# toposware/schnorr-sig

Measured on AMD Instinct MI355X. Metric: Schnorr verifications/sec, 2^20-sig batch, 1/2/4/8 MI355X; bit-exact vs CPU, higher is better.
Workload: dtype u64

## Files before the change

schnorr-sig_amd/csrc/fp6.hpp:

```cpp
#pragma once
#include "fp.hpp"

namespace ssa {

#if defined(__HIP_DEVICE_COMPILE__) && !defined(SSA_NO_F6_ASM)
#define SSA_F6_ASM 1
#include "fp6_asm.inc"
#endif

struct fp6 {
    u64 c[6];
};

SSA_DEV fp6 f6_zero() {
    fp6 r;
#pragma unroll
    for (int i = 0; i < 6; i++) r.c[i] = 0ull;
    return r;
}
SSA_DEV fp6 f6_one() {
    fp6 r = f6_zero();
    r.c[0] = 1ull;
    return r;
}
// ... 125 lines not shown
}

SSA_FN fp6 f6_sqr_flat(u64 a0, u64 a1, u64 a2_, u64 a3, u64 a4, u64 a5) {
    fp6 a;
    a.c[0] = a0; a.c[1] = a1; a.c[2] = a2_; a.c[3] = a3; a.c[4] = a4; a.c[5] = a5;
    u64 a2[6], a7[6], a14[6];
    f6_sqr_scale(a.c, a2, a7, a14);
#ifdef SSA_F6_ASM
    fp6 r;
    f6_sqr_core_asm(a.c, a2, a7, a14, r.c);
    return r;
#else
    fp6 r;
#pragma unroll
    for (int k = 0; k < 6; k++) {
        fp_acc s;
        bool first = true;
#pragma unroll
        for (int i = 0; i <= k / 2; i++) {
            int j = k - i;
            u64 y = (i == j) ? a.c[j] : a2[j];
            if (first) {
                acc_init(s, a.c[i], y);
                first = false;
            } else {
                acc_mac(s, a.c[i], y);
            }
        }
#pragma unroll
        for (int i = k + 1; i <= (k + 6) / 2; i++) {
            int j = k + 6 - i;
            if (j > 5) continue;
            u64 y = (i == j) ? a7[j] : a14[j];
            acc_mac(s, a.c[i], y);
        }
        r.c[k] = acc_reduce(s);
    }
    return r;
#endif
}
SSA_DEV fp6 f6_sqr(const fp6 &a) { return f6_sqr_flat(a.c[0], a.c[1], a.c[2], a.c[3], a.c[4], a.c[5]); }

SSA_DEV fp6 f6_sqr_inl(const fp6 &a) {
#ifdef SSA_F6_ASM
    u64 a2[6], a7[6], a14[6];
    f6_sqr_scale(a.c, a2, a7, a14);
    fp6 r;
    f6_sqr_core_asm(a.c, a2, a7, a14, r.c);
    return r;
#else
    return f6_sqr(a);
#endif
}

SSA_DEV void f6_sqr_prescale(const fp6 &a, u64 (&a2)[6], u64 (&a7)[6], u64 (&a14)[6]) {
    f6_sqr_scale(a.c, a2, a7, a14);
}
SSA_DEV void f6_mul_prescale(const fp6 &b, u64 (&b7)[6]) {
    b7[0] = 0ull;
#pragma unroll
    for (int j = 1; j < 6; j++) b7[j] = fp_mul_small(b.c[j], 7u);
}
SSA_DEV fp6 f6_sqr_sub2(const fp6 &a, const fp6 &x, const fp6 &y) {
#ifdef SSA_F6_ASM
    u64 a2[6], a7[6], a14[6];
    f6_sqr_prescale(a, a2, a7, a14);
    fp6 r;
    f6_sqr_sub2_core_asm(a.c, a2, a7, a14, x.c, y.c, r.c);
    return r;
#else
    return f6_sub(f6_sub(f6_sqr(a), x), y);
#endif
}
SSA_DEV fp6 f6_sqr_subx_sub2y(const fp6 &a, const fp6 &x, const fp6 &y) {
#ifdef SSA_F6_ASM
    u64 a2[6], a7[6], a14[6];
    f6_sqr_prescale(a, a2, a7, a14);
    fp6 r;
    f6_sqr_subx_sub2y_core_asm(a.c, a2, a7, a14, x.c, y.c, r.c);
    return r;
#else
    return f6_sub(f6_sub(f6_sqr(a), x), f6_dbl(y));
#endif
}
SSA_DEV fp6 f6_sqr_add3x(const fp6 &a, const fp6 &x) {
#ifdef SSA_F6_ASM
    u64 a2[6], a7[6], a14[6];
    f6_sqr_prescale(a, a2, a7, a14);
    fp6 r;
    f6_sqr_add3x_core_asm(a.c, a2, a7, a14, x.c, r.c);
    return r;
#else
    return f6_add(f6_sqr(a), f6_add(f6_dbl(x), x));
#endif
}
SSA_DEV fp6 f6_sqr_sub4x(const fp6 &a, const fp6 &x) {
#ifdef SSA_F6_ASM
    u64 a2[6], a7[6], a14[6];
    f6_sqr_prescale(a, a2, a7, a14);
    fp6 r;
    f6_sqr_sub4x_core_asm(a.c, a2, a7, a14, x.c, r.c);
    return r;
#else
    return f6_sub(f6_sqr(a), f6_dbl(f6_dbl(x)));
#endif
}
// ... 110 lines not shown
```

schnorr-sig_amd/csrc/ssa_api.hip:

```cpp
#define SSA_KERNELS_DEFINE 1
#include "ssa_ctx.hpp"
#include "ssa_keycache.hpp"
#include "ssa_keyed.hpp"

#include <sys/random.h>

#include <atomic>
#include <climits>
#include <functional>
#include <initializer_list>
#include <memory>
#include <mutex>
#include <thread>

static const unsigned char k_default_params[SSA_PARAMS_LENGTH] = {
#include "../params/params_default.inc"
};

extern "C" const char *ssa_strerror(int rc) {
    switch (rc) {
        case SSA_OK: return "ok";
        case SSA_INVALID_PUBLIC_KEY: return "The public key is not an element of the prime subgroup.";
        case SSA_INVALID_SIGNATURE: return "The signature is invalid or was incorrectly computed.";
        case SSA_MALFORMED: return "malformed input (the reference would panic)";
// ... 431 lines not shown
    if (int rc = check_msgs(mv, n)) return rc;
    if (n == 0) return 0;
    HIP_TRY(hipSetDevice(ctx->device));
    return timed_launch(ctx, "ssa_k_hash", [&] {
        hipLaunchKernelGGL(ssa_k_hash, dim3(grid_for(n, 256)), dim3(256), 0, ctx->stream, ctx->d_params,
                           d_sigs, d_pks, mv, n, (u64 *)nullptr, d_digests_out, (const u32 *)nullptr, 0u);
    });
}

extern "C" int ssa_rescue_hash_many_device(ssa_ctx *ctx, const uint64_t *d_felts, uint32_t felts_per_row,
                                           size_t n, uint64_t *d_digests_out) {
    if (!ctx || (n && (!d_digests_out || (felts_per_row && !d_felts)))) return SSA_ERR_ARG;
    if (n == 0) return 0;
    HIP_TRY(hipSetDevice(ctx->device));
    return timed_launch(ctx, "ssa_k_rescue", [&] {
        hipLaunchKernelGGL(ssa_k_rescue, dim3(grid_for(n, 256)), dim3(256), 0, ctx->stream, ctx->d_params,
                           (const u64 *)d_felts, felts_per_row, n, (u64 *)d_digests_out);
    });
}

int ssa_internal_hash_chunk(ssa_ctx *ctx, hipStream_t hs, const DevBatch &b, size_t cnt, uint64_t *d_h) {
    hipLaunchKernelGGL(ssa_k_hash, dim3(grid_for(cnt, 256)), dim3(256), 0, hs, ctx->d_params, b.sigs, b.pks, b.msgs, cnt,
                       (u64 *)d_h, (u8 *)nullptr, (const u32 *)nullptr, 0u);
    HIP_TRY(hipGetLastError());
    return 0;
}

int ssa_internal_hash_scalars(ssa_ctx *ctx, const DevBatch &b, size_t n) {
    if (ctx->ws_h.reserve(n * 4 * sizeof(u64))) return SSA_ERR_HIP;
    return timed_launch(ctx, "ssa_k_hash", [&] {
        hipLaunchKernelGGL(ssa_k_hash, dim3(grid_for(n, 256)), dim3(256), 0, ctx->stream, ctx->d_params,
                           b.sigs, b.pks, b.msgs, n, (u64 *)ctx->ws_h.p, (u8 *)nullptr, (const u32 *)nullptr, 0u);
    });
}

struct TailKnobs {
    unsigned pieces, gens, waves, block, min_main;
    bool uniform, reversed;
};
static TailPlan tail_plan_of(const TailKnobs &kn, size_t cnt, uint32_t flags) {
    const TailKnobs *ctx = &kn;
    TailPlan tp{};
    const bool torsion = (flags & SSA_FLAG_CHECK_TORSION) != 0;
    tp.whole[0] = 0u | 2u | 4u | ((u32)LADDER_STEPS_Q << 16);
    tp.whole[1] = 1u | 2u | 4u | ((u32)LADDER_STEPS << 16);
    const u32 n_groups = (u32)((cnt + 63) / 64);
    const unsigned cap = torsion ? (unsigned)VP_MAX - 1u : (unsigned)VP_MAX;
    const unsigned want = ctx->pieces < cap ? ctx->pieces : cap;
    const u32 tail0 = ctx->gens * ctx->waves;
    if (want < 2 || ctx->block != 256 || tail0 == 0 || n_groups < tail0 + ctx->min_main * ctx->waves) return tp;
    const u32 main_groups = ((n_groups - tail0) / 4u) * 4u;
    tp.main_blocks = main_groups / 4u;
    tp.tail_groups = ((n_groups - main_groups + 3u) / 4u) * 4u;
    const double DBL = 2642.0, ADD = 3738.0, TABLE = 57000.0, TAIL = 45000.0;
    struct Step { int pass, it; double cost; };
    std::vector<Step> steps;
    for (int pass = torsion ? 0 : 1; pass < 2; pass++)
        for (int it = 0; it < (pass == 0 ? LADDER_STEPS_Q : LADDER_STEPS); it++)
            steps.push_back({pass, it, (pass == 0 ? (double)QNAF_GAP[it + 1] : 5.0) * DBL + ADD});
    double total = TABLE + TAIL;
    for (const Step &st : steps) total += st.cost;
    std::vector<double> target;
    double frac = 0.0, f = 0.5;
    for (unsigned k = 0; k + 1 < want; k++) {
        frac += ctx->uniform ? 1.0 / (double)want : f;
        if (k + 2 < want) f *= 0.5;
        target.push_back(total * frac);
    }
    std::vector<std::pair<size_t, size_t>> pieces;
    size_t cur = 0, tix = 0;
    double acc = TABLE;
    for (size_t idx = 0; idx < steps.size(); idx++) {
        bool cut = false;
        if (idx > cur) {
            if (steps[idx].pass != steps[idx - 1].pass) cut = true;
            else if (tix < target.size() && acc + steps[idx].cost * 0.5 >= target[tix]) cut = true;
        }
        if (cut) {
            pieces.push_back({cur, idx});
            cur = idx;
        }
        while (tix < target.size() && acc + steps[idx].cost * 0.5 >= target[tix]) tix++;
        acc += steps[idx].cost;
    }
    pieces.push_back({cur, steps.size()});
    if (pieces.size() < 2 || pieces.size() > (size_t)VP_MAX) return tp;
    for (const auto &pc : pieces) {
        const int pass = steps[pc.first].pass, lo = steps[pc.first].it, hi = steps[pc.second - 1].it + 1;
        const int n_steps = pass == 0 ? LADDER_STEPS_Q : LADDER_STEPS;
        tp.ph[tp.n_pieces++] = (u32)pass | (lo == 0 ? 2u : 0u) | (hi == n_steps ? 4u : 0u) | ((u32)lo << 8) | ((u32)hi << 16);
    }
    tp.reversed = ctx->reversed ? 1u : 0u;
    return tp;
}
static TailPlan tail_plan(const ssa_ctx *ctx, size_t cnt, uint32_t flags) {
    return tail_plan_of({ctx->knobs.tail_pieces, ctx->knobs.tail_gens, ctx->knobs.verify_waves, ctx->knobs.verify_block, ctx->knobs.tail_min_main,
                         ctx->knobs.tail_uniform, ctx->knobs.tail_reversed}, cnt, flags);
}

extern "C" int ssa_debug_tail_plan(unsigned waves, unsigned pieces, unsigned gens, int uniform, unsigned min_main, size_t n,
                                   uint32_t flags, uint32_t out[14]) {
    if (!out) return SSA_ERR_ARG;
    const TailPlan tp = tail_plan_of({pieces, gens, waves, 256u, min_main, uniform != 0, false}, n, flags);
    out[0] = tp.n_pieces;
    out[1] = tp.tail_groups;
    out[2] = tp.main_blocks;
    out[3] = tp.n_pieces ? tail_grid_blocks(tp) : (uint32_t)((n + 255) / 256);
    for (int k = 0; k < VP_MAX; k++) out[4 + k] = tp.ph[k];
    out[12] = tp.whole[0];
    out[13] = tp.whole[1];
    return 0;
}

static int verify_slices(ssa_ctx *ctx, const DevBatch &b, const u64 *d_h, size_t n, uint32_t flags, uint8_t *d_status_out,
                         unsigned long long *d_fail) {
    return for_dev_slices(b, n, ctx->knobs.lane_slice, [&](size_t lo, size_t cnt, const DevBatch &s) {
        const TailPlan tp = tail_plan(ctx, cnt, flags);
        unsigned blocks = grid_for(cnt, ctx->knobs.verify_block);
        if (tp.n_pieces) {
            if (ctx->tail_done.reserve(2 * (size_t)tp.tail_groups * sizeof(u32)) ||
                ctx->tail_park.reserve((size_t)tp.tail_groups * PARK_WORDS * 64 * sizeof(u64)))
                return SSA_ERR_HIP;
            HIP_TRY(hipMemsetAsync(ctx->tail_done.p, 0, 2 * (size_t)tp.tail_groups * sizeof(u32), ctx->stream));
            blocks = tail_grid_blocks(tp);
        }
        return timed_launch(ctx, "ssa_k_verify", [&] {
            hipLaunchKernelGGL(ssa_k_verify, dim3(blocks), dim3(ctx->knobs.verify_block), 0,
                               ctx->stream, s.sigs, s.pks, s.pk_inf, d_h + 4 * lo, (const u64 *)ctx->d_gtab,
                               (u64 *)ctx->ws_tab.p, cnt, flags, d_status_out + lo, d_fail, tp, (u32 *)ctx->tail_done.p,
                               (u64 *)ctx->tail_park.p);
        });
    });
}

int ssa_internal_verify_hashed(ssa_ctx *ctx, const DevBatch &b, const uint64_t *d_h, size_t n, uint32_t flags,
                               uint8_t *d_status_out, unsigned long long *d_fail) {
    const size_t slice = ctx->knobs.lane_slice < n ? ctx->knobs.lane_slice : n;
    if (ctx->ws_tab.reserve(slice * (size_t)(PTAB_ENTRIES * PTAB_ENTRY_U64) * sizeof(u64))) return SSA_ERR_HIP;
    return verify_slices(ctx, b, (const u64 *)d_h, n, flags, d_status_out, d_fail);
}

static int verify_one_slice(ssa_ctx *c, const DevBatch &b, size_t cnt, uint32_t flags, uint8_t *d_status_out,
                            unsigned long long *d_fail) {
    if (c->ws_h.reserve(cnt * 4 * sizeof(u64))) return SSA_ERR_HIP;
    if (c->ws_tab.reserve(cnt * (size_t)(PTAB_ENTRIES * PTAB_ENTRY_U64) * sizeof(u64))) return SSA_ERR_HIP;
    int rc = timed_launch(c, "ssa_k_hash", [&] {
        hipLaunchKernelGGL(ssa_k_hash, dim3(grid_for(cnt, 256)), dim3(256), 0, c->stream, c->d_params, b.sigs, b.pks,
                           b.msgs, cnt, (u64 *)c->ws_h.p, (u8 *)nullptr, (const u32 *)nullptr, 0u);
    });
    if (rc) return rc;
    return verify_slices(c, b, (const u64 *)c->ws_h.p, cnt, flags, d_status_out, d_fail);
}

static int verify_launch(ssa_ctx *ctx, const DevBatch &b, size_t n, uint32_t flags, uint8_t *d_status_out,
                         unsigned long long *d_fail) {
    if (takes_coop(ctx, n, flags)) {
        return timed_launch(ctx, "ssa_k_verify_coop", [&] {
            hipLaunchKernelGGL(ssa_k_verify_coop, dim3((unsigned)n), dim3(128), 0, ctx->stream, ctx->d_params, b.sigs,
                               b.pks, b.pk_inf, b.msgs, (const u64 *)ctx->d_gtab, n, flags, d_status_out, d_fail);
        });
    }
    const size_t slice = ctx->knobs.lane_slice < n ? ctx->knobs.lane_slice : n;
    if (n <= slice) return verify_one_slice(ctx, b, n, flags, d_status_out, d_fail);
    ssa_ctx *tw = ssa_internal_twin(ctx);
    if (tw) {
        HIP_TRY(hipEventRecord(ctx->order_ev, ctx->stream));
        HIP_TRY(hipStreamWaitEvent(tw->stream, ctx->order_ev, 0));
    }
    int rc = 0;
    size_t j = 0;
    for (size_t lo = 0; lo < n && rc == 0; lo += slice, j++) {
        const size_t cnt = n - lo < slice ? n - lo : slice;
        ssa_ctx *c = (tw && (j & 1u)) ? tw : ctx;
        rc = verify_one_slice(c, b.slice(lo), cnt, flags, d_status_out + lo, d_fail);
    }
    if (tw) {
        if (hipEventRecord(tw->order_ev, tw->stream) != hipSuccess ||
            hipStreamWaitEvent(ctx->stream, tw->order_ev, 0) != hipSuccess)
            return rc ? rc : SSA_ERR_HIP;
    }
    return rc;
}

// ... 1232 lines not shown
```

schnorr-sig_amd/csrc/ssa_ctx.hpp:

```cpp
#pragma once
#include "../../include/schnorr_sig_amd.h"
#include "ssa_kernels.hpp"

#include <hip/hip_runtime.h>

#include <algorithm>
#include <cstdio>
#include <cstdlib>
#include <cstring>
#include <map>
#include <mutex>
#include <string>
#include <thread>
#include <utility>
#include <vector>

using namespace ssa;

static inline bool ssa_debug_enabled() {
    static const bool on = std::getenv("SSA_DEBUG") != nullptr;
    return on;
}
#define HIP_TRY(expr)                                                                    \
    do {                                                                                 \
// ... 41 lines not shown
    size_t cap = 0;
    int reserve(size_t bytes) {
        if (bytes <= cap) return 0;
        if (p) (void)hipHostFree(p);
        p = nullptr;
        cap = 0;
        const size_t want = bytes + bytes / 8 + 4096;
        if (hipHostMalloc(&p, want, hipHostMallocDefault) != hipSuccess) {
            (void)hipGetLastError();
            p = nullptr;
            return SSA_ERR_HIP;
        }
        cap = want;
        return 0;
    }
    void release() {
        if (p) (void)hipHostFree(p);
        p = nullptr;
        cap = 0;
    }
};

struct TimedLaunch {
    hipEvent_t start, stop;
};

constexpr double DEDUP_RATIO_NO_CHECK = 0.0, DEDUP_RATIO_CHECK = 1.0;
constexpr unsigned DEDUP_PROBE_BOUND = 128;

struct CtxKnobs {
    size_t pipeline_min_n = 1 << 17;
    unsigned pipeline_chunks = 8;
    size_t coop_max_n = 7680, coop_max_n_torsion = 10496;
    size_t msm_small_max = 3072;
    size_t lane_slice = (size_t)1 << 20, msm_slice = (size_t)1 << 23;
    bool msm_overlap = true;
    unsigned msm_tree_group = 16;
    unsigned verify_block = 256;
    unsigned verify_waves = 0;
    unsigned tail_pieces = 5;
    unsigned tail_gens = 1;
    bool tail_uniform = false;
    bool tail_reversed = false;
    unsigned tail_min_main = 0;
    unsigned tail_waves_override = 0;
    bool timing = false;
    unsigned screen_segs = 0;
    double dedup_ratio[2] = {DEDUP_RATIO_NO_CHECK, DEDUP_RATIO_CHECK};
    unsigned dedup_probe_bound = DEDUP_PROBE_BOUND;
};

#define SSA_CTX_DEVBUFS(X) \
    X(ws_h) X(ws_tab) X(ws_fail) \
     \
    X(st_sigs) X(st_pks) X(st_inf) X(st_msgs) X(st_off) X(st_status) X(st_aux) X(st_aux2) X(st_coeffs) \
     \
    X(msm_points) X(msm_scalars) X(msm_keys) X(msm_vals) X(msm_keys2) X(msm_vals2) X(msm_sort_tmp) X(msm_bounds) \
    X(msm_buckets) X(msm_chunks) X(msm_windows) X(msm_partials) X(msm_flags) X(msm_cnt) X(msm_cnt2) X(msm_ids) \
    X(msm_ids2) X(msm_comb_pts) X(msm_comb_lins) \
    X(msm_slice_recs)    \
    X(msm_sbuf)          \
     \
    X(scr_ok) X(scr_in) X(scr_status) X(scr_fail) \
     \
    X(scr_mask) X(scr_mark) X(scr_list) X(scr_blk) X(scr_cnt) \
     \
    X(dd_slots) X(dd_rep) X(dd_num) X(dd_reps) X(dd_idx) X(dd_blk) X(dd_stats) X(dd_pks) X(dd_inf) X(dd_kstatus) \
     \
    X(kc_found) X(kc_missrep) X(kc_blk) X(kc_lane_row) \
     \
    X(st_keyed) X(ky_sigs) X(ky_pks) X(ky_inf) \
     \
    X(ctab) X(sg_sigs) X(sg_pks) \
    X(tc_out)            \
    X(kck_ws)            \
    X(dv_recs)           \
     \
    X(rng_seed) X(rng_scratch) \
     \
    X(tail_done) X(tail_park)

#define SSA_CTX_HOSTBUFS(X) X(pin_in) X(pin_coeffs) X(pin_out) X(pin_seed)

struct ssa_ctx {
    int device = 0;
    hipStream_t own_stream = nullptr;
    hipStream_t stream = nullptr;
    hipStream_t copy_stream = nullptr;
    hipEvent_t copy_done[8] = {};
    hipStream_t hash_stream[2] = {};
    hipEvent_t hash_done[8] = {};
    hipEvent_t pipe_start = nullptr;
    hipEvent_t order_ev = nullptr;
    CtxKnobs knobs;
    DevParams *d_params = nullptr;
    u64 *d_gtab = nullptr;
    struct SharedGtab *gtab_share = nullptr;
    uint32_t gtab_bits = 0;
    uint64_t hbm_budget = 0;
    DevParams h_params;
    ssa_ctx *twin = nullptr;
    bool is_twin = false, two_streams = true;
#define X(name) DevBuf name;
    SSA_CTX_DEVBUFS(X)
#undef X
#define X(name) HostBuf name;
// ... 553 lines not shown
```

schnorr-sig_amd/csrc/ssa_kernels.hpp:

```cpp
#pragma once
#include "curve.hpp"
#include "fp3.hpp"
#include "rescue.hpp"

namespace ssa {

struct GtabGeom {
    u32 bits, count;
};
constexpr int GW_BITS_MAX = 24, GW_BITS_MIN = 16;
__host__ __device__ inline u32 gtab_windows(u32 bits) { return (255u + bits) / bits; }
__host__ __device__ inline size_t gtab_entries(u32 bits) { return (size_t)gtab_windows(bits) << bits; }
__host__ __device__ inline size_t gbase_entries(u32 bits) { return ((size_t)gtab_windows(bits) * 2) << (bits / 2); }
__host__ __device__ inline u64 gtab_header(u32 bits) { return (u64)bits | ((u64)gtab_windows(bits) << 8); }
SSA_DEV GtabGeom gtab_geom(const u64 *__restrict__ gtab) {
    const u32 v = (u32)__builtin_amdgcn_readfirstlane((int)(u32)gtab[0]);
    GtabGeom g;
    g.bits = v & 0xffu;
    g.count = (v >> 8) & 0xffu;
    return g;
}
constexpr int PTAB_ENTRIES = 16;
constexpr int PTAB_ENTRY_U64 = 32, PTAB_Z = 16, PTAB_C = 22;
constexpr int PTAB_NEG = 16, PTAB_NY = PTAB_NEG + 6;
// ... 169 lines not shown
        ulonglong2 a = q[i], b = q[3 + i], c = q[6 + i];
        p.X.c[2 * i] = a.x; p.X.c[2 * i + 1] = a.y;
        p.Y.c[2 * i] = b.x; p.Y.c[2 * i + 1] = b.y;
        p.Z.c[2 * i] = c.x; p.Z.c[2 * i + 1] = c.y;
    }
    return p;
}
SSA_DEV aff ld_aff(const u64 *__restrict__ row) {
    const ulonglong2 *q = reinterpret_cast<const ulonglong2 *>(row);
    aff p;
#pragma unroll
    for (int i = 0; i < 3; i++) {
        ulonglong2 a = q[i], b = q[3 + i];
        p.x.c[2 * i] = a.x; p.x.c[2 * i + 1] = a.y;
        p.y.c[2 * i] = b.x; p.y.c[2 * i + 1] = b.y;
    }
    return p;
}

SSA_DEV void st_f6(u64 *__restrict__ p, const fp6 &a) {
    ulonglong2 *q = reinterpret_cast<ulonglong2 *>(p);
#pragma unroll
    for (int i = 0; i < 3; i++) q[i] = make_ulonglong2(a.c[2 * i], a.c[2 * i + 1]);
}
SSA_DEV fp6 ld_f6(const u64 *__restrict__ p) {
    const ulonglong2 *q = reinterpret_cast<const ulonglong2 *>(p);
    fp6 a;
#pragma unroll
    for (int i = 0; i < 3; i++) {
        ulonglong2 v = q[i];
        a.c[2 * i] = v.x;
        a.c[2 * i + 1] = v.y;
    }
    return a;
}
SSA_DEV void st_aff(u64 *__restrict__ row, const aff &p) {
    st_f6(row, p.x);
    st_f6(row + 6, p.y);
}

SSA_DEV void st_row(u64 *__restrict__ row, const jac &p) {
    st_f6(row, p.X);
    st_f6(row + 6, p.Y);
    st_f6(row + PTAB_Z, p.Z);
}
SSA_DEV jac ld_row(const u64 *__restrict__ row) {
    jac p;
    p.X = ld_f6(row);
    p.Y = ld_f6(row + 6);
    p.Z = ld_f6(row + PTAB_Z);
    return p;
}

SSA_FN void tab_dbl(u64 *__restrict__ dst, const u64 *__restrict__ src) { st_row(dst, jac_dbl(ld_row(src))); }
SSA_FN void tab_madd(u64 *__restrict__ dst, const u64 *__restrict__ src, const u64 *__restrict__ paff) {
    st_row(dst, jac_madd(ld_row(src), ld_aff(paff)));
}

SSA_DEV fp6 aff_dbl_num(const fp6 &x) {
    const fp6 xx = f6_sqr(x);
    fp6 n = f6_add(f6_dbl(xx), xx);
    n.c[0] = fp_add(n.c[0], 1ull);
    return n;
}
SSA_DEV aff aff_from_slope(const fp6 &l, const fp6 &x1, const fp6 &y1, const fp6 &x2) {
    aff r;
    r.x = f6_sub(f6_sub(f6_sqr(l), x1), x2);
    r.y = f6_sub(f6_mul(l, f6_sub(x1, r.x)), y1);
    return r;
}
SSA_DEV void st_tab_entry(u64 *__restrict__ row, const aff &a) {
    st_aff(row, a);
    st_f6(row + PTAB_NEG, a.x);
    st_f6(row + PTAB_NY, f6_neg(a.y));
}
SSA_DEV bool build_ptab_affine_upper(u64 *__restrict__ tab) {
    constexpr int R = PTAB_ENTRY_U64;
    const aff p8 = ld_aff(tab + 7 * R);
    fp6 c = f6_one();
#pragma unroll 1
    for (int m = 9; m <= 16; m++) {
        const aff b = ld_aff(tab + (((m & 1) ? m - 8 : m / 2) - 1) * R);
        const fp6 d = (m & 1) ? f6_sub(p8.x, b.x) : f6_dbl(b.y);
        st_f6(tab + (m - 1) * R + PTAB_Z, d);
        c = f6_mul(c, d);
        st_f6(tab + (m - 1) * R + PTAB_C, c);
    }
    if (f6_is_zero(c)) return false;
    fp6 inv = f6_inv(c);
#pragma unroll 1
    for (int m = 16; m >= 9; m--) {
        fp6 di = inv;
        if (m > 9) di = f6_mul(inv, ld_f6(tab + (m - 2) * R + PTAB_C));
        inv = f6_mul(inv, ld_f6(tab + (m - 1) * R + PTAB_Z));
        const aff b = ld_aff(tab + (((m & 1) ? m - 8 : m / 2) - 1) * R);
        aff r;
        if (m & 1) r = aff_from_slope(f6_mul(f6_sub(p8.y, b.y), di), b.x, b.y, p8.x);
        else r = aff_from_slope(f6_mul(aff_dbl_num(b.x), di), b.x, b.y, b.x);
        st_tab_entry(tab + (m - 1) * R, r);
    }
    return true;
}

SSA_DEV bool build_ptab_affine(u64 *__restrict__ tab, const aff &p) {
    constexpr int R = PTAB_ENTRY_U64;
    const fp6 d2 = f6_dbl(p.y);
    if (f6_is_zero(d2)) return false;
    const aff p2 = aff_from_slope(f6_mul(aff_dbl_num(p.x), f6_inv(d2)), p.x, p.y, p.x);
    const fp6 a3 = f6_sub(p2.x, p.x), a4 = f6_dbl(p2.y);
    const fp6 t34 = f6_mul(a3, a4);
    if (f6_is_zero(t34)) return false;
    const fp6 i34 = f6_inv(t34);
    const aff p3 = aff_from_slope(f6_mul(f6_sub(p2.y, p.y), f6_mul(i34, a4)), p.x, p.y, p2.x);
    const aff p4 = aff_from_slope(f6_mul(aff_dbl_num(p2.x), f6_mul(i34, a3)), p2.x, p2.y, p2.x);
    const fp6 a5 = f6_sub(p4.x, p.x), a6 = f6_dbl(p3.y), a7 = f6_sub(p4.x, p3.x), a8 = f6_dbl(p4.y);
    const fp6 t56 = f6_mul(a5, a6), t567 = f6_mul(t56, a7), t5678 = f6_mul(t567, a8);
    if (f6_is_zero(t5678)) return false;
    fp6 inv = f6_inv(t5678);
    const fp6 i8 = f6_mul(inv, t567);
    inv = f6_mul(inv, a8);
    const fp6 i7 = f6_mul(inv, t56);
    inv = f6_mul(inv, a7);
    const fp6 i6 = f6_mul(inv, a5), i5 = f6_mul(inv, a6);
    st_tab_entry(tab, p);
    st_tab_entry(tab + 1 * R, p2);
    st_tab_entry(tab + 2 * R, p3);
    st_tab_entry(tab + 3 * R, p4);
    st_tab_entry(tab + 4 * R, aff_from_slope(f6_mul(f6_sub(p4.y, p.y), i5), p.x, p.y, p4.x));
    st_tab_entry(tab + 5 * R, aff_from_slope(f6_mul(aff_dbl_num(p3.x), i6), p3.x, p3.y, p3.x));
    st_tab_entry(tab + 6 * R, aff_from_slope(f6_mul(f6_sub(p4.y, p3.y), i7), p3.x, p3.y, p4.x));
    st_tab_entry(tab + 7 * R, aff_from_slope(f6_mul(aff_dbl_num(p4.x), i8), p4.x, p4.y, p4.x));
    return build_ptab_affine_upper(tab);
}

SSA_DEV void build_ptab(u64 *__restrict__ tab, const aff &p, bool p_inf) {
    constexpr int R = PTAB_ENTRY_U64;
    if (p_inf) {
        aff z;
        z.x = f6_zero();
        z.y = f6_zero();
#pragma unroll 1
        for (int e = 0; e < PTAB_ENTRIES; e++) st_tab_entry(tab + e * R, z);
        return;
    }
#ifndef SSA_PTAB_JACOBIAN_ONLY
    if (build_ptab_affine(tab, p)) return;
#endif
    st_row(tab, jac_from_aff(p));
    tab_dbl(tab + 1 * R, tab);
    tab_madd(tab + 2 * R, tab + 1 * R, tab);
    tab_dbl(tab + 3 * R, tab + 1 * R);
    tab_madd(tab + 4 * R, tab + 3 * R, tab);
    tab_dbl(tab + 5 * R, tab + 2 * R);
    tab_madd(tab + 6 * R, tab + 5 * R, tab);
    tab_dbl(tab + 7 * R, tab + 3 * R);
#pragma unroll 1
    for (int m = 9; m <= 16; m++) {
        if (m & 1) tab_madd(tab + (m - 1) * R, tab + (m - 2) * R, tab);
        else tab_dbl(tab + (m - 1) * R, tab + (m / 2 - 1) * R);
    }
    fp6 c = f6_one();
#pragma unroll 1
    for (int e = 1; e < PTAB_ENTRIES; e++) {
        fp6 z = ld_f6(tab + e * R + PTAB_Z);
        if (f6_is_zero(z)) z = f6_one();
        c = f6_mul(c, z);
        st_f6(tab + e * R + PTAB_C, c);
    }
    fp6 inv = f6_inv(c);
#pragma unroll 1
    for (int e = PTAB_ENTRIES - 1; e >= 1; e--) {
        fp6 z = ld_f6(tab + e * R + PTAB_Z);
        const bool zero = f6_is_zero(z);
        if (zero) z = f6_one();
        fp6 zinv = inv;
        if (e > 1) zinv = f6_mul(inv, ld_f6(tab + (e - 1) * R + PTAB_C));
        inv = f6_mul(inv, z);
        const fp6 zi2 = f6_sqr(zinv);
        aff a;
        a.x = f6_mul(ld_f6(tab + e * R), zi2);
        a.y = f6_mul(ld_f6(tab + e * R + 6), f6_mul(zi2, zinv));
        if (zero) {
            a.x = f6_zero();
            a.y = f6_zero();
        }
        st_tab_entry(tab + e * R, a);
    }
    st_tab_entry(tab, p);
}

#include "qnaf.inc"

constexpr int LADDER_STEPS = 50, LADDER_STEPS_Q = QNAF_LEN - 1;
SSA_DEV jac ladder_init(const u64 *__restrict__ tab, const sc256 &kr, bool order_q) {
    jac acc = jac_identity();
    const u32 top = order_q ? (u32)QNAF_DIGIT[0] : sc_top5(kr);
    if (top != 0) {
        const aff p = ld_aff(tab + ((top > 16u ? 16u : top) - 1u) * PTAB_ENTRY_U64);
        if (!(f6_is_zero(p.x) && f6_is_zero(p.y))) acc = jac_from_aff(p);
        if (top > 16u) acc = jac_madd_fast(acc, ld_aff(tab + (top - 17u) * PTAB_ENTRY_U64));
    }
    return acc;
}
SSA_DEV jac ladder_steps(jac acc, const u64 *&tab, const sc256 &kr, bool order_q, int lo, int hi) {
#pragma unroll 1
    for (int it = lo; it < hi; it++) {
        int digit;
        u32 gap;
        if (order_q) {
            digit = (int)QNAF_DIGIT[it + 1];
            gap = (u32)QNAF_GAP[it + 1];
        } else {
// ... 102 lines not shown
    u32 n_pieces;
    u32 tail_groups;
    u32 main_blocks;
    u32 ph[VP_MAX];
    u32 whole[2];
    u32 reversed;
};
__host__ __device__ inline u32 tail_grid_blocks(const TailPlan &tp) { return tp.main_blocks + tp.n_pieces * (tp.tail_groups / 4u); }
struct BlockRole {
    u32 piece;
    u32 index;
};
SSA_DEV BlockRole tail_role(const TailPlan &tp, u32 blk) {
    BlockRole r;
    r.piece = 0xffffffffu;
    r.index = blk;
    if (tp.n_pieces == 0) return r;
    const u32 pb = tp.tail_groups / 4u;
    if (blk < pb) {
        r.piece = 0;
        return r;
    }
    if (blk < pb + tp.main_blocks) {
        r.index = blk - pb;
        return r;
    }
    const u32 q = blk - pb - tp.main_blocks;
    r.piece = 1u + q / pb;
    r.index = q - (r.piece - 1u) * pb;
    return r;
}
constexpr int PARK_WORDS = 19;
SSA_DEV void st_shared(u64 *__restrict__ p, u64 v) { __hip_atomic_store(p, v, __ATOMIC_RELAXED, __HIP_MEMORY_SCOPE_AGENT); }
SSA_DEV void park_store(u64 *__restrict__ pk, const jac &r) {
#pragma unroll
    for (int k = 0; k < 6; k++) {
        st_shared(pk + k * 64, r.X.c[k]);
        st_shared(pk + (6 + k) * 64, r.Y.c[k]);
        st_shared(pk + (12 + k) * 64, r.Z.c[k]);
    }
}
SSA_DEV jac park_load(const u64 *__restrict__ pk) {
    jac r;
#pragma unroll
    for (int k = 0; k < 6; k++) {
        r.X.c[k] = pk[k * 64];
        r.Y.c[k] = pk[(6 + k) * 64];
        r.Z.c[k] = pk[(12 + k) * 64];
    }
    return r;
}

#ifndef SSA_NO_KERNELS
__global__ void __launch_bounds__(256, 2)
ssa_k_verify(const u8 *__restrict__ sigs, const u8 *__restrict__ pks,
             const u8 *__restrict__ pk_inf, const u64 *__restrict__ h_in,
             const u64 *__restrict__ gtab, u64 *__restrict__ ws_tab, size_t n, u32 flags,
             u8 *__restrict__ status_out, unsigned long long *__restrict__ n_fail,
             TailPlan tp, u32 *__restrict__ done, u64 *__restrict__ park) {
#ifdef SSA_WAVE_TIMES
    const unsigned long long wt0 = wall_clock64();
#endif
    const BlockRole role = tail_role(tp, tp.reversed ? gridDim.x - 1u - blockIdx.x : blockIdx.x);
    const u32 lane = threadIdx.x & 63u;
    const bool in_piece = role.piece != 0xffffffffu;
    const u32 p_lo = in_piece ? role.piece : 0u;
    const u32 eg = in_piece ? 4u * role.index + (threadIdx.x >> 6) : 0u;
    const size_t i = in_piece ? ((size_t)tp.main_blocks * 256u + (size_t)eg * 64u + lane)
                              : ((size_t)role.index * blockDim.x + threadIdx.x);
    const bool runs_last = !in_piece || p_lo + 1u == tp.n_pieces;
    const bool in = i < n;
    u64 *pk = park + ((size_t)eg * PARK_WORDS) * 64 + lane;
    u64 *tab = ws_tab + i * (size_t)(PTAB_ENTRIES * PTAB_ENTRY_U64);
    u32 status = ST_OK;
    bool ok_sig = true;
    jac r = jac_identity();
    u32 run_lo = p_lo;
    if (in_piece) {
        u32 *next = done + tp.tail_groups + eg;
        u32 cur = 0;
        if (lane == 0) {
            cur = __hip_atomic_load(next, __ATOMIC_RELAXED, __HIP_MEMORY_SCOPE_AGENT);
            while (cur <= p_lo) {
                const u32 seen = atomicCAS(next, cur, p_lo + 1u);
                if (seen == cur) break;
                cur = seen;
            }
        }
        cur = (u32)__builtin_amdgcn_readfirstlane((int)cur);
        if (cur > p_lo) return;
        run_lo = cur;
    }
    if (in_piece && run_lo > 0) {
        while (__hip_atomic_load(done + eg, __ATOMIC_RELAXED, __HIP_MEMORY_SCOPE_AGENT) < run_lo) __builtin_amdgcn_s_sleep(64);
        __builtin_amdgcn_fence(__ATOMIC_ACQUIRE, "agent");
        asm volatile("s_waitcnt vmcnt(0)" ::: "memory");
        const u64 sw = pk[18 * 64];
        status = (u32)(sw & 0xffu);
        ok_sig = ((sw >> 8) & 1u) != 0;
        if (in && status == ST_OK && !(tp.ph[run_lo] & 2u)) r = park_load(pk);
    } else if (in) {
        bool ok = true;
        const fp6 xs = ld_fp6(sigs + 81 * i, ok_sig);
        const sc256 e = ld_sc(sigs + 81 * i + 49);
        ok_sig = ok_sig && !sc_geq_q(e);
        const u32 fbyte = sigs[81 * i + 48];
        if ((flags & VF_SIG_FLAG_BYTE) && ok_sig) ok_sig = sig_flag_precheck(fbyte, f6_is_zero(xs)) == ST_OK;
        aff P;
        P.x = ld_fp6(pks + 96 * i, ok);
        P.y = ld_fp6(pks + 96 * i + 48, ok);
        const bool inf = pk_inf && pk_inf[i];
        if (ok && !inf) ok = aff_on_curve(P);
        if (!ok) status = ST_MALFORMED;
        else build_ptab(tab, P, inf);
    }
    SSA_PHASE_MARK(1);
    if (in && status == ST_OK) {
        sc256 h;
#pragma unroll
        for (int k = 0; k < 4; k++) h.w[k] = h_in[4 * i + k];
        const sc256 kr = sc_recode_offset5(h);
        const u32 d_lo = in_piece ? run_lo : ((flags & VF_CHECK_TORSION) ? 0u : 1u);
        const u32 d_hi = in_piece ? p_lo + 1u : 2u;
        const u64 *ltab = tab;
#pragma unroll 1
        for (u32 k = d_lo; k < d_hi; k++) {
            const u32 d = in_piece ? tp.ph[k] : tp.whole[k];
            const bool pass_q = (d & 1u) == 0, first = (d & 2u) != 0, last = (d & 4u) != 0;
            if (first) {
                if (!pass_q && !ok_sig) {
                    status = ST_MALFORMED;
                    break;
                }
                r = ladder_init(ltab, kr, pass_q);
            }
            r = ladder_steps(r, ltab, kr, pass_q, (int)((d >> 8) & 0xffu), (int)((d >> 16) & 0xffu));
            if (last && pass_q && !jac_is_identity(r)) {
                status = ST_INVALID_PK;
                break;
            }
        }
    }
    SSA_PHASE_MARK(2);
    if (runs_last) {
        if (in) {
            if (status == ST_OK) {
                bool okx = true;
                const fp6 xs = ld_fp6(sigs + 81 * i, okx);
                const sc256 e = ld_sc(sigs + 81 * i + 49);
                const u32 fbyte = sigs[81 * i + 48];
#ifdef SSA_COMB_HOT
                r = add_base_mul(r, gtab, e, true);
#else
                r = add_base_mul(r, gtab, e);
#endif
                bool eq;
                if (flags & VF_SIG_FLAG_BYTE) {
                    if (fbyte & 0x80u) {
                        eq = jac_is_identity(r);
                    } else {
                        eq = !jac_is_identity(r) && f6_eq(r.X, f6_mul(xs, f6_sqr(r.Z)));
                        if (eq) eq = jac_y_lex_largest(r) == ((fbyte & 0x40u) != 0);
#ifndef SSA_COMB_HOT
                        else if (!x_on_curve(xs)) ok_sig = false;
#endif
                    }
                } else if (jac_is_identity(r)) {
// ... 915 lines not shown
```

Measured before the change: 30.65 million.

## Split public-key table construction into a separate higher-occupancy kernel

Moves public-key parsing, the on-curve check and the per-key precompute table build out of the verify kernel into a new ssa_k_ptab kernel launched just before it. That kernel runs at launch bounds of 4 blocks per CU instead of 2, and it passes a per-lane status byte through a new workspace buffer. The tail-planner's table cost is set to zero because the verify kernel no longer builds the table. The cost is an extra launch, plus the table now being written and read back through global memory across two kernels. Templated inline-versus-call field-arithmetic policies are added, but the call path stays the default.

```diff
diff --git a/schnorr-sig_amd/csrc/fp6.hpp b/schnorr-sig_amd/csrc/fp6.hpp
--- a/schnorr-sig_amd/csrc/fp6.hpp
+++ b/schnorr-sig_amd/csrc/fp6.hpp
@@ -201,6 +201,27 @@
     return f6_sqr(a);
 #endif
 }
+SSA_DEV fp6 f6_mul_inl(const fp6 &a, const fp6 &b) {
+#ifdef SSA_F6_ASM
+    u64 b7[6];
+    b7[0] = 0ull;
+#pragma unroll
+    for (int j = 1; j < 6; j++) b7[j] = fp_mul_small(b.c[j], 7u);
+    fp6 r;
+    f6_mul_core_asm(a.c, b.c, b7, r.c);
+    return r;
+#else
+    return f6_mul(a, b);
+#endif
+}
+struct F6Call {
+    static SSA_DEV fp6 mul(const fp6 &a, const fp6 &b) { return f6_mul(a, b); }
+    static SSA_DEV fp6 sqr(const fp6 &a) { return f6_sqr(a); }
+};
+struct F6Inline {
+    static SSA_DEV fp6 mul(const fp6 &a, const fp6 &b) { return f6_mul_inl(a, b); }
+    static SSA_DEV fp6 sqr(const fp6 &a) { return f6_sqr_inl(a); }
+};
 
 SSA_DEV void f6_sqr_prescale(const fp6 &a, u64 (&a2)[6], u64 (&a7)[6], u64 (&a14)[6]) {
     f6_sqr_scale(a.c, a2, a7, a14);
diff --git a/schnorr-sig_amd/csrc/ssa_api.hip b/schnorr-sig_amd/csrc/ssa_api.hip
--- a/schnorr-sig_amd/csrc/ssa_api.hip
+++ b/schnorr-sig_amd/csrc/ssa_api.hip
@@ -507,7 +507,7 @@
     const u32 main_groups = ((n_groups - tail0) / 4u) * 4u;
     tp.main_blocks = main_groups / 4u;
     tp.tail_groups = ((n_groups - main_groups + 3u) / 4u) * 4u;
-    const double DBL = 2642.0, ADD = 3738.0, TABLE = 57000.0, TAIL = 45000.0;
+    const double DBL = 2642.0, ADD = 3738.0, TABLE = 0.0, TAIL = 45000.0;
     struct Step { int pass, it; double cost; };
     std::vector<Step> steps;
     for (int pass = torsion ? 0 : 1; pass < 2; pass++)
@@ -579,11 +579,14 @@
             HIP_TRY(hipMemsetAsync(ctx->tail_done.p, 0, 2 * (size_t)tp.tail_groups * sizeof(u32), ctx->stream));
             blocks = tail_grid_blocks(tp);
         }
+        if (ctx->ws_kstat.reserve(cnt)) return SSA_ERR_HIP;
         return timed_launch(ctx, "ssa_k_verify", [&] {
+            hipLaunchKernelGGL(ssa_k_ptab, dim3(grid_for(cnt, 256)), dim3(256), 0, ctx->stream, s.pks, s.pk_inf,
+                               (u64 *)ctx->ws_tab.p, (u8 *)ctx->ws_kstat.p, cnt);
             hipLaunchKernelGGL(ssa_k_verify, dim3(blocks), dim3(ctx->knobs.verify_block), 0,
-                               ctx->stream, s.sigs, s.pks, s.pk_inf, d_h + 4 * lo, (const u64 *)ctx->d_gtab,
-                               (u64 *)ctx->ws_tab.p, cnt, flags, d_status_out + lo, d_fail, tp, (u32 *)ctx->tail_done.p,
-                               (u64 *)ctx->tail_park.p);
+                               ctx->stream, s.sigs, (const u8 *)ctx->ws_kstat.p, d_h + 4 * lo, (const u64 *)ctx->d_gtab,
+                               (const u64 *)ctx->ws_tab.p, cnt, flags, d_status_out + lo, d_fail, tp,
+                               (u32 *)ctx->tail_done.p, (u64 *)ctx->tail_park.p);
         });
     });
 }
diff --git a/schnorr-sig_amd/csrc/ssa_ctx.hpp b/schnorr-sig_amd/csrc/ssa_ctx.hpp
--- a/schnorr-sig_amd/csrc/ssa_ctx.hpp
+++ b/schnorr-sig_amd/csrc/ssa_ctx.hpp
@@ -117,6 +117,7 @@
 
 #define SSA_CTX_DEVBUFS(X) \
     X(ws_h) X(ws_tab) X(ws_fail) \
+    X(ws_kstat)          \
      \
     X(st_sigs) X(st_pks) X(st_inf) X(st_msgs) X(st_off) X(st_status) X(st_aux) X(st_aux2) X(st_coeffs) \
      \
diff --git a/schnorr-sig_amd/csrc/ssa_kernels.hpp b/schnorr-sig_amd/csrc/ssa_kernels.hpp
--- a/schnorr-sig_amd/csrc/ssa_kernels.hpp
+++ b/schnorr-sig_amd/csrc/ssa_kernels.hpp
@@ -245,21 +245,25 @@
     return p;
 }
 
+template <class F = F6Call>
 SSA_FN void tab_dbl(u64 *__restrict__ dst, const u64 *__restrict__ src) { st_row(dst, jac_dbl(ld_row(src))); }
+template <class F = F6Call>
 SSA_FN void tab_madd(u64 *__restrict__ dst, const u64 *__restrict__ src, const u64 *__restrict__ paff) {
     st_row(dst, jac_madd(ld_row(src), ld_aff(paff)));
 }
 
+template <class F = F6Call>
 SSA_DEV fp6 aff_dbl_num(const fp6 &x) {
-    const fp6 xx = f6_sqr(x);
+    const fp6 xx = F::sqr(x);
     fp6 n = f6_add(f6_dbl(xx), xx);
     n.c[0] = fp_add(n.c[0], 1ull);
     return n;
 }
+template <class F = F6Call>
 SSA_DEV aff aff_from_slope(const fp6 &l, const fp6 &x1, const fp6 &y1, const fp6 &x2) {
     aff r;
-    r.x = f6_sub(f6_sub(f6_sqr(l), x1), x2);
-    r.y = f6_sub(f6_mul(l, f6_sub(x1, r.x)), y1);
+    r.x = f6_sub(f6_sub(F::sqr(l), x1), x2);
+    r.y = f6_sub(F::mul(l, f6_sub(x1, r.x)), y1);
     return r;
 }
 SSA_DEV void st_tab_entry(u64 *__restrict__ row, const aff &a) {
@@ -267,6 +271,7 @@
     st_f6(row + PTAB_NEG, a.x);
     st_f6(row + PTAB_NY, f6_neg(a.y));
 }
+template <class F = F6Call>
 SSA_DEV bool build_ptab_affine_upper(u64 *__restrict__ tab) {
     constexpr int R = PTAB_ENTRY_U64;
     const aff p8 = ld_aff(tab + 7 * R);
@@ -276,7 +281,7 @@
         const aff b = ld_aff(tab + (((m & 1) ? m - 8 : m / 2) - 1) * R);
         const fp6 d = (m & 1) ? f6_sub(p8.x, b.x) : f6_dbl(b.y);
         st_f6(tab + (m - 1) * R + PTAB_Z, d);
-        c = f6_mul(c, d);
+        c = F::mul(c, d);
         st_f6(tab + (m - 1) * R + PTAB_C, c);
     }
     if (f6_is_zero(c)) return false;
@@ -284,48 +289,50 @@
 #pragma unroll 1
     for (int m = 16; m >= 9; m--) {
         fp6 di = inv;
-        if (m > 9) di = f6_mul(inv, ld_f6(tab + (m - 2) * R + PTAB_C));
-        inv = f6_mul(inv, ld_f6(tab + (m - 1) * R + PTAB_Z));
+        if (m > 9) di = F::mul(inv, ld_f6(tab + (m - 2) * R + PTAB_C));
+        inv = F::mul(inv, ld_f6(tab + (m - 1) * R + PTAB_Z));
         const aff b = ld_aff(tab + (((m & 1) ? m - 8 : m / 2) - 1) * R);
         aff r;
-        if (m & 1) r = aff_from_slope(f6_mul(f6_sub(p8.y, b.y), di), b.x, b.y, p8.x);
-        else r = aff_from_slope(f6_mul(aff_dbl_num(b.x), di), b.x, b.y, b.x);
+        if (m & 1) r = aff_from_slope<F>(F::mul(f6_sub(p8.y, b.y), di), b.x, b.y, p8.x);
+        else r = aff_from_slope<F>(F::mul(aff_dbl_num<F>(b.x), di), b.x, b.y, b.x);
         st_tab_entry(tab + (m - 1) * R, r);
     }
     return true;
 }
 
+template <class F = F6Call>
 SSA_DEV bool build_ptab_affine(u64 *__restrict__ tab, const aff &p) {
     constexpr int R = PTAB_ENTRY_U64;
     const fp6 d2 = f6_dbl(p.y);
     if (f6_is_zero(d2)) return false;
-    const aff p2 = aff_from_slope(f6_mul(aff_dbl_num(p.x), f6_inv(d2)), p.x, p.y, p.x);
+    const aff p2 = aff_from_slope<F>(F::mul(aff_dbl_num<F>(p.x), f6_inv(d2)), p.x, p.y, p.x);
     const fp6 a3 = f6_sub(p2.x, p.x), a4 = f6_dbl(p2.y);
-    const fp6 t34 = f6_mul(a3, a4);
+    const fp6 t34 = F::mul(a3, a4);
     if (f6_is_zero(t34)) return false;
     const fp6 i34 = f6_inv(t34);
-    const aff p3 = aff_from_slope(f6_mul(f6_sub(p2.y, p.y), f6_mul(i34, a4)), p.x, p.y, p2.x);
-    const aff p4 = aff_from_slope(f6_mul(aff_dbl_num(p2.x), f6_mul(i34, a3)), p2.x, p2.y, p2.x);
+    const aff p3 = aff_from_slope<F>(F::mul(f6_sub(p2.y, p.y), F::mul(i34, a4)), p.x, p.y, p2.x);
+    const aff p4 = aff_from_slope<F>(F::mul(aff_dbl_num<F>(p2.x), F::mul(i34, a3)), p2.x, p2.y, p2.x);
     const fp6 a5 = f6_sub(p4.x, p.x), a6 = f6_dbl(p3.y), a7 = f6_sub(p4.x, p3.x), a8 = f6_dbl(p4.y);
-    const fp6 t56 = f6_mul(a5, a6), t567 = f6_mul(t56, a7), t5678 = f6_mul(t567, a8);
+    const fp6 t56 = F::mul(a5, a6), t567 = F::mul(t56, a7), t5678 = F::mul(t567, a8);
     if (f6_is_zero(t5678)) return false;
     fp6 inv = f6_inv(t5678);
-    const fp6 i8 = f6_mul(inv, t567);
-    inv = f6_mul(inv, a8);
-    const fp6 i7 = f6_mul(inv, t56);
-    inv = f6_mul(inv, a7);
-    const fp6 i6 = f6_mul(inv, a5), i5 = f6_mul(inv, a6);
+    const fp6 i8 = F::mul(inv, t567);
+    inv = F::mul(inv, a8);
+    const fp6 i7 = F::mul(inv, t56);
+    inv = F::mul(inv, a7);
+    const fp6 i6 = F::mul(inv, a5), i5 = F::mul(inv, a6);
     st_tab_entry(tab, p);
     st_tab_entry(tab + 1 * R, p2);
     st_tab_entry(tab + 2 * R, p3);
     st_tab_entry(tab + 3 * R, p4);
-    st_tab_entry(tab + 4 * R, aff_from_slope(f6_mul(f6_sub(p4.y, p.y), i5), p.x, p.y, p4.x));
-    st_tab_entry(tab + 5 * R, aff_from_slope(f6_mul(aff_dbl_num(p3.x), i6), p3.x, p3.y, p3.x));
-    st_tab_entry(tab + 6 * R, aff_from_slope(f6_mul(f6_sub(p4.y, p3.y), i7), p3.x, p3.y, p4.x));
-    st_tab_entry(tab + 7 * R, aff_from_slope(f6_mul(aff_dbl_num(p4.x), i8), p4.x, p4.y, p4.x));
-    return build_ptab_affine_upper(tab);
-}
-
+    st_tab_entry(tab + 4 * R, aff_from_slope<F>(F::mul(f6_sub(p4.y, p.y), i5), p.x, p.y, p4.x));
+    st_tab_entry(tab + 5 * R, aff_from_slope<F>(F::mul(aff_dbl_num<F>(p3.x), i6), p3.x, p3.y, p3.x));
+    st_tab_entry(tab + 6 * R, aff_from_slope<F>(F::mul(f6_sub(p4.y, p3.y), i7), p3.x, p3.y, p4.x));
+    st_tab_entry(tab + 7 * R, aff_from_slope<F>(F::mul(aff_dbl_num<F>(p4.x), i8), p4.x, p4.y, p4.x));
+    return build_ptab_affine_upper<F>(tab);
+}
+
+template <class F = F6Call>
 SSA_DEV void build_ptab(u64 *__restrict__ tab, const aff &p, bool p_inf) {
     constexpr int R = PTAB_ENTRY_U64;
     if (p_inf) {
@@ -337,20 +344,20 @@
         return;
     }
 #ifndef SSA_PTAB_JACOBIAN_ONLY
-    if (build_ptab_affine(tab, p)) return;
+    if (build_ptab_affine<F>(tab, p)) return;
 #endif
     st_row(tab, jac_from_aff(p));
-    tab_dbl(tab + 1 * R, tab);
-    tab_madd(tab + 2 * R, tab + 1 * R, tab);
-    tab_dbl(tab + 3 * R, tab + 1 * R);
-    tab_madd(tab + 4 * R, tab + 3 * R, tab);
-    tab_dbl(tab + 5 * R, tab + 2 * R);
-    tab_madd(tab + 6 * R, tab + 5 * R, tab);
-    tab_dbl(tab + 7 * R, tab + 3 * R);
+    tab_dbl<F>(tab + 1 * R, tab);
+    tab_madd<F>(tab + 2 * R, tab + 1 * R, tab);
+    tab_dbl<F>(tab + 3 * R, tab + 1 * R);
+    tab_madd<F>(tab + 4 * R, tab + 3 * R, tab);
+    tab_dbl<F>(tab + 5 * R, tab + 2 * R);
+    tab_madd<F>(tab + 6 * R, tab + 5 * R, tab);
+    tab_dbl<F>(tab + 7 * R, tab + 3 * R);
 #pragma unroll 1
     for (int m = 9; m <= 16; m++) {
-        if (m & 1) tab_madd(tab + (m - 1) * R, tab + (m - 2) * R, tab);
-        else tab_dbl(tab + (m - 1) * R, tab + (m / 2 - 1) * R);
+        if (m & 1) tab_madd<F>(tab + (m - 1) * R, tab + (m - 2) * R, tab);
+        else tab_dbl<F>(tab + (m - 1) * R, tab + (m / 2 - 1) * R);
     }
     fp6 c = f6_one();
 #pragma unroll 1
@@ -559,10 +566,33 @@
 }
 
 #ifndef SSA_NO_KERNELS
+#ifndef SSA_PTAB_OCC
+#define SSA_PTAB_OCC 4
+#endif
+#ifdef SSA_PTAB_INLINE
+using PtabF6 = F6Inline;
+#else
+struct F6CallPtab : F6Call {};
+using PtabF6 = F6CallPtab;
+#endif
+__global__ void __launch_bounds__(256, SSA_PTAB_OCC)
+ssa_k_ptab(const u8 *__restrict__ pks, const u8 *__restrict__ pk_inf, u64 *__restrict__ ws_tab, u8 *__restrict__ kstat,
+           size_t n) {
+    const size_t i = (size_t)blockIdx.x * blockDim.x + threadIdx.x;
+    if (i >= n) return;
+    bool ok = true;
+    aff P;
+    P.x = ld_fp6(pks + 96 * i, ok);
+    P.y = ld_fp6(pks + 96 * i + 48, ok);
+    const bool inf = pk_inf && pk_inf[i];
+    if (ok && !inf) ok = aff_on_curve(P);
+    if (ok) build_ptab<PtabF6>(ws_tab + i * (size_t)(PTAB_ENTRIES * PTAB_ENTRY_U64), P, inf);
+    kstat[i] = (u8)(ok ? ST_OK : ST_MALFORMED);
+}
+
 __global__ void __launch_bounds__(256, 2)
-ssa_k_verify(const u8 *__restrict__ sigs, const u8 *__restrict__ pks,
-             const u8 *__restrict__ pk_inf, const u64 *__restrict__ h_in,
-             const u64 *__restrict__ gtab, u64 *__restrict__ ws_tab, size_t n, u32 flags,
+ssa_k_verify(const u8 *__restrict__ sigs, const u8 *__restrict__ kstat, const u64 *__restrict__ h_in,
+             const u64 *__restrict__ gtab, const u64 *__restrict__ ws_tab, size_t n, u32 flags,
              u8 *__restrict__ status_out, unsigned long long *__restrict__ n_fail,
              TailPlan tp, u32 *__restrict__ done, u64 *__restrict__ park) {
 #ifdef SSA_WAVE_TIMES
@@ -578,7 +608,7 @@
     const bool runs_last = !in_piece || p_lo + 1u == tp.n_pieces;
     const bool in = i < n;
     u64 *pk = park + ((size_t)eg * PARK_WORDS) * 64 + lane;
-    u64 *tab = ws_tab + i * (size_t)(PTAB_ENTRIES * PTAB_ENTRY_U64);
+    const u64 *tab = ws_tab + i * (size_t)(PTAB_ENTRIES * PTAB_ENTRY_U64);
     u32 status = ST_OK;
     bool ok_sig = true;
     jac r = jac_identity();
@@ -607,19 +637,12 @@
         ok_sig = ((sw >> 8) & 1u) != 0;
         if (in && status == ST_OK && !(tp.ph[run_lo] & 2u)) r = park_load(pk);
     } else if (in) {
-        bool ok = true;
         const fp6 xs = ld_fp6(sigs + 81 * i, ok_sig);
         const sc256 e = ld_sc(sigs + 81 * i + 49);
         ok_sig = ok_sig && !sc_geq_q(e);
         const u32 fbyte = sigs[81 * i + 48];
         if ((flags & VF_SIG_FLAG_BYTE) && ok_sig) ok_sig = sig_flag_precheck(fbyte, f6_is_zero(xs)) == ST_OK;
-        aff P;
-        P.x = ld_fp6(pks + 96 * i, ok);
-        P.y = ld_fp6(pks + 96 * i + 48, ok);
-        const bool inf = pk_inf && pk_inf[i];
-        if (ok && !inf) ok = aff_on_curve(P);
-        if (!ok) status = ST_MALFORMED;
-        else build_ptab(tab, P, inf);
+        if (kstat[i] != (u8)ST_OK) status = ST_MALFORMED;
     }
     SSA_PHASE_MARK(1);
     if (in && status == ST_OK) {
```

Measured after the change: 28.44 million. 0.928x the previous value.
